# jkaardal/pyipm

Measured on AMD Instinct MI355X. Metric: newton_steps_per_sec, higher is better.
Workload: dtype f64

## Files before the change

### pyipm_amd/csrc/ctx.hpp

```cpp
#pragma once
#include <hip/hip_runtime.h>
#include <stdint.h>
#include <stdio.h>
#include <stdlib.h>
#include <string.h>
#include <string>
#include <new>
#include <stdexcept>
#include <map>
#include <memory>
#include <vector>
#include "../../include/pyipm_newton.h"
#include "owned.hpp"
#include "step_plan.hpp"

namespace pyipm {

constexpr int TB = PYIPM_TILE;
static_assert(TB == PLAN_TB, "step_plan.hpp states the tile on its own");
constexpr int PADG = PYIPM_PAD;
constexpr int BM = 128;
constexpr int BKU = 16;
constexpr int ROWCHUNK = 2048;

// ... 198 lines not shown
    struct TileList { unsigned* dev = nullptr; unsigned count = 0;
                      Event ready; hipStream_t on = nullptr; bool seen_done = false; };
    struct TlArena { DevBuf<unsigned> dev; PinnedBuf<unsigned> host{hipHostMallocDefault}; size_t used = 0; };
    std::vector<TlArena> tl_arenas;
    std::map<std::vector<int64_t>, TileList> tile_lists;
    int skip_zeros = 1;
    int group = 1;
    bool tail_group_user = false;
    int tail_group = 4;
    GroupSched sched;
    double* Wnext = nullptr;
    int group_chain = 1;
    Stream rest;
    std::vector<Event> ev_band;
    Event ev_join, ev_main, ev_split, ev_sfast;
    int keep_zeros = 1;
    int tile_step = 1;
    int sweep_max_blocks = 0;
    int occ_fwd_sweep = 0, occ_bwd_sweep = 0, occ_fwd_prefix = 0, occ_fwd_range = 0;
    int sweep_persist = 1;
    int bwd_slack = 1;
    DevBuf<double> sweep_buf;
    DevBuf<double> ms_buf;
    DevBuf<double> km_buf;
    int ms_matvec_many = 0;
    PollWords sweep_words{3 * 4096,
                          "backward sweep (k_bwd_sweep): a poll timed out in an earlier solve; its result was NaN"};
    int dist_slices = 2;
    double dist_timeout_s = 300.0;
    int dist_comm2 = 0;
// ... 157 lines not shown
```

### pyipm_amd/csrc/pyipm_newton.hip

```cpp
#include "driver.hpp"
#include "sub_walk.hpp"
#include "kernels_assemble.hpp"
#include "kernels_factor.hpp"
#include "kernels_panel.hpp"
#include "kernels_chain.hpp"
#include "kernels_solve.hpp"
#include "kernels_msolve.hpp"
#include "kernels_kmany.hpp"
#include "kernels_batched.hpp"
#include "kernels_merit.hpp"

using namespace pyipm;
using namespace pyipm::drv;

namespace pyipm { namespace drv {


size_t carve_workspace(Ctx* c, const Geo& g, char* base, bool provider_only = false) {
    Carve cv;
    const size_t D = sizeof(double);
    const size_t oA = cv.take(provider_only ? 256 : (size_t)g.Npad * (size_t)(g.ncols_local > 0 ? g.ncols_local : 1) * D);
    const size_t oW = cv.take(provider_only ? 256 : 3 * (size_t)default_group(g.world, g.nb) * (size_t)g.Npad * g.nb * D);
    const size_t oL = cv.take(g.world > 1 ? (size_t)g.Npad * g.nb * D : 256);
    const size_t oD = cv.take(provider_only ? 256 : (size_t)(g.Npad / TB) * TB * TB * D);
// ... 493 lines not shown
            hipLaunchKernelGGL(k_tile_step8, dim3(nblk), dim3(512), 0, chain, ctx->A, g.Npad, gc0, glc0, j, nT, ny, upb,
                               Wg, g.Npad, Dv, Ts, ctx->Tflag + gc0 / TB, ctx->refine_cond, ctx->block_refine, ctx->dstats, g.N,
                               ctx->pivtol_rel, ctx->anorm, g.n + g.mi, ctx->dbg_buf, ctx->tile_blocked);
            PYIPM_KCHECK();
            continue;
        }
        hipLaunchKernelGGL(k_tile_step, dim3((unsigned)(nT - j), (unsigned)ny), dim3(256), 0, chain, ctx->A, g.Npad, gc0, glc0, j,
                           Wg, g.Npad, Dv, Ts, ctx->Tflag + gc0 / TB, ctx->refine_cond, ctx->block_refine, ctx->dstats, g.N,
                           ctx->pivtol_rel, ctx->anorm, g.n + g.mi, ctx->dbg_buf, ctx->tile_blocked);
        PYIPM_KCHECK();
    }
    return 0;
}

struct SubPanel { int64_t c0, lc0; int nt; double* W; int64_t id; };
struct BlockDesc {
    std::vector<SubPanel> sp;
    bool wide = false;
    int64_t lp = 0;
    int64_t hole0 = 0, hole1 = 0;
};
int factor_block(Ctx* ctx, const BlockDesc& bd, hipStream_t chain, const std::function<int(int64_t, hipStream_t)>& on_done) {
    const Geo& g = ctx->g;
    const int64_t n0 = (int64_t)bd.sp.size();
    std::vector<int> toff((size_t)n0 + 1, 0);
    for (int64_t k = 0; k < n0; ++k) toff[(size_t)k + 1] = toff[(size_t)k] + bd.sp[(size_t)k].nt;
    const int nT = toff[(size_t)n0];
    const int64_t gc0 = bd.sp[0].c0, glc0 = bd.sp[0].lc0, gend = gc0 + (int64_t)nT * TB;
    const int64_t TT = (int64_t)TB * TB;
    { int r0 = ensure_rest_stream(ctx); if (r0) return r0; }
    PYIPM_HIP(ctx->ev_join.ensure(hipEventDisableTiming));
    PYIPM_HIP(ensure_events(ctx->ev_band, (size_t)n0, hipEventDisableTiming));
    double* Wg = bd.sp[0].W;
    double* Dv = ctx->Dinv + (gc0 / TB) * TT;
    double* Ts = ctx->Tsv + (gc0 / TB) * TT;
    auto upd = [&](hipStream_t st, const double* Lop, const double* Wop, int K, int64_t row_begin, int64_t k1, int64_t cnt,
                   int64_t src_c0) -> int {
        if (!bd.wide)
            return launch_update128(ctx, st, Lop, g.Npad, Wop, K, row_begin, bd.sp[(size_t)k1].id, cnt, {.bulk = false, .src_c0 = src_c0});
        const int s0 = (int)((bd.sp[(size_t)k1].c0 - g.panel_c0(bd.lp * g.world + g.rank)) / 128);
        const int nc = (int)((int64_t)(toff[(size_t)(k1 + cnt)] - toff[(size_t)k1]) * TB / 128);
        return launch_update128(ctx, st, Lop, g.Npad, Wop, K, row_begin, bd.lp, 1,
                                {.bulk = false, .src_c0 = src_c0, .sub0 = s0, .nct_sub = nc});
    };
    const bool one_launch = ctx->chain_whole && chain_applies(ctx, gc0, nT);
    ChainGeo cgw; memset(&cgw, 0, sizeof(cgw));
    if (one_launch) {
        PYIPM_HIP(hipEventRecord(ctx->ev_band[0], chain));
        PYIPM_HIP(hipStreamWaitEvent(ctx->rest, ctx->ev_band[0], 0));
        int r0 = launch_tile_steps(ctx, chain, gc0, glc0, nT, 0, nT, Wg, Dv, Ts); if (r0) return r0;
        cgw = ctx->chain_last;
    }
    for (int kp = 1, ta = 0; kp <= n0 && !one_launch; ++kp) {
        const int tb = kp < n0 ? toff[(size_t)kp] + 1 : nT;
        int r0 = launch_tile_steps(ctx, chain, gc0, glc0, nT, ta, tb, Wg, Dv, Ts); if (r0) return r0;
        if (kp < n0) PYIPM_HIP(hipEventRecord(ctx->ev_band[(size_t)(kp - 1)], chain));
        ta = tb;
    }
    for (int64_t k = 0; k < n0; ++k) {
        const SubPanel& q = bd.sp[(size_t)k];
        const int64_t c0 = q.c0, lc0 = q.lc0;
        const int nt = q.nt;
        hipStream_t rs = ctx->rest;
        if (k + 1 == n0) {
            PYIPM_HIP(hipEventRecord(ctx->ev_join, ctx->rest));
            PYIPM_HIP(hipStreamWaitEvent(chain, ctx->ev_join, 0));
            rs = chain;
        } else if (one_launch) {
            hipLaunchKernelGGL(k_chain_wait, dim3(1), dim3(64), 0, ctx->rest, cgw, toff[(size_t)k + 1], toff[(size_t)k + 1], toff[(size_t)k + 1]);
            PYIPM_KCHECK();
        } else {
            PYIPM_HIP(hipStreamWaitEvent(ctx->rest, ctx->ev_band[(size_t)k], 0));
        }
        const bool left = g.Npad - gend > PENDING_LEFT_ROWS;
        if (g.Npad > gend && left && k > 0) {
            const int K = toff[(size_t)k] * TB;
            int rc = upd(rs, ctx->A + glc0 * g.Npad, Wg, K, gend, k, 1, gc0);
            if (rc) return rc;
        }
        if (g.Npad > gend) {
            hipLaunchKernelGGL(k_panel_rest, dim3((unsigned)((g.Npad - gend) / TB)), dim3(256), 0, rs, ctx->A, g.Npad, c0, lc0, nt,
                               gend, q.W, g.Npad, ctx->Dinv + (c0 / TB) * TT, ctx->Tsv + (c0 / TB) * TT, ctx->Tflag + c0 / TB,
                               ctx->block_refine, bd.hole0, bd.hole1, &ctx->dstats->growth_bits);
            PYIPM_KCHECK();
            if (k + 1 < n0 && !left) {
                const int K = nt * TB;
                const SubPanel& nx = bd.sp[(size_t)k + 1];
                const int64_t tc0 = nx.c0, ncols = (int64_t)(nT - toff[(size_t)k + 1]) * TB;
                if (g.Npad - tc0 <= PENDING32_ROWS) {
                    int64_t pa0, pa1, pb0, pb1;
                    active_ranges(ctx, c0, c0 + K, &pa0, &pa1, &pb0, &pb1);
                    hipLaunchKernelGGL(k_inpanel_update, dim3((unsigned)((g.Npad - gend) / 32), (unsigned)(ncols / TB)), dim3(256), 0,
                                       rs, ctx->A, g.Npad, nx.lc0, ctx->A + lc0 * g.Npad, g.Npad, q.W, g.Npad,
                                       tc0, K, gend, g.Npad, pa0, pa1, pb0, pb1, SIDE_PRIO);
                    PYIPM_KCHECK();
                } else {
                    int rc = upd(rs, ctx->A + lc0 * g.Npad, q.W, K, gend, k + 1, n0 - 1 - k, c0);
                    if (rc) return rc;
                }
            }
        }
        if (one_launch && k + 1 < n0) {
            const int tq = toff[(size_t)k + 1] + 1;
            hipLaunchKernelGGL(k_chain_wait, dim3(1), dim3(64), 0, ctx->rest, cgw, tq, tq, tq);
            PYIPM_KCHECK();
        }
        int rc = on_done(q.id, rs); if (rc) return rc;
    }
    return 0;
}

int factor_group(Ctx* ctx, int64_t p0, int64_t n0, hipStream_t chain, const std::function<int(int64_t, hipStream_t)>& on_done) {
    const Geo& g = ctx->g;
    BlockDesc bd;
    for (int64_t k = 0; k < n0; ++k) {
        const int64_t q = p0 + k;
        bd.sp.push_back(SubPanel{g.panel_c0(q), g.local_c0(q), (int)(g.panel_w(q) / TB), wbuf(ctx, q), q});
    }
    if (ctx->skip_zeros && g.mi > 0 && ctx->sched.in_x_panel(p0)) slack_hole(g, &bd.hole0, &bd.hole1);
    return factor_block(ctx, bd, chain, on_done);
}

int factor_wide_panel(Ctx* ctx, int64_t p, hipStream_t stream) {
    const Geo& g = ctx->g;
    const int64_t c0 = g.panel_c0(p), lc0 = g.local_c0(p);
    const int nt = (int)(g.panel_w(p) / TB), snt = ctx->wide_sub / TB;
    BlockDesc bd;
    bd.wide = true; bd.lp = p / g.world;
    double* W = wbuf(ctx, p);
// ... 8 lines not shown
bool panel_is_wide(const Ctx* ctx, int64_t p) {
    return ctx->wide_sub >= 128 && ctx->wide_sub % 128 == 0 && ctx->g.panel_w(p) > ctx->wide_sub;
}
bool panel_piecewise_ok(const Ctx* ctx, int64_t p) {
    if (!ctx->tile_step || panel_in_s(ctx, p)) return false;
    const int nt = (int)ctx->g.panel_w(p) / TB;
    return panel_is_wide(ctx, p) ? (nt <= 32) : (nt <= 16);
}
int panel_chain(Ctx* ctx, int64_t p, hipStream_t stream, int64_t xrows, const unsigned* xword, unsigned xwant) {
    const Geo& g = ctx->g;
    const int64_t c0 = g.panel_c0(p), lc0 = g.local_c0(p);
    const int nt = (int)(g.panel_w(p) / TB);
    return launch_tile_steps(ctx, stream, c0, lc0, nt, 0, nt, wbuf(ctx, p), ctx->Dinv + (c0 / TB) * (int64_t)(TB * TB),
                             ctx->Tsv + (c0 / TB) * (int64_t)(TB * TB), (int)(xrows / TB), xword, xwant);
}
bool chain_extra_ok(const Ctx* ctx, int64_t p, int64_t xrows) {
    const Geo& g = ctx->g;
    const int64_t c0 = g.panel_c0(p);
    const int nbw = (int)g.panel_w(p), nt = nbw / TB;
    if (xrows <= 0 || xrows % TB != 0 || xrows / TB > 16 || c0 + nbw + xrows > g.Npad) return false;
    if (!(nt >= 2 && chain_applies(ctx, c0, nt))) return false;
    if (1 + 4 * (nt + (int)(xrows / TB)) > Ctx::CHAIN_WORDS) return false;
    int64_t h0 = 0, h1 = 0;
    panel_hole(ctx, p, &h0, &h1);
    const int64_t r0 = c0 + nbw, r1 = r0 + xrows;
    return !(h1 > h0 && r1 > h0 && r0 < h1);
}
int panel_rows(Ctx* ctx, int64_t p, int64_t r0, int64_t r1, hipStream_t stream) {
    const Geo& g = ctx->g;
    if (r1 > g.Npad) r1 = g.Npad;
    if (r1 <= r0) return 0;
    const int64_t c0 = g.panel_c0(p), lc0 = g.local_c0(p), TT = (int64_t)TB * TB;
    const int nbw = (int)g.panel_w(p), nt = nbw / TB;
    double* W = wbuf(ctx, p);
    int64_t hole0 = 0, hole1 = 0;
    panel_hole(ctx, p, &hole0, &hole1);
    if (!panel_is_wide(ctx, p)) {
        hipLaunchKernelGGL(k_panel_rest, dim3((unsigned)((r1 - r0) / TB)), dim3(256), 0, stream, ctx->A, g.Npad, c0, lc0, nt, r0,
                           W, g.Npad, ctx->Dinv + (c0 / TB) * TT, ctx->Tsv + (c0 / TB) * TT, ctx->Tflag + c0 / TB,
                           ctx->block_refine, hole0, hole1, &ctx->dstats->growth_bits);
        PYIPM_KCHECK();
// ... 885 lines not shown

static int panel_done(Ctx* ctx, const FactorRun& run, int64_t grp, int64_t q, hipStream_t used) {
    if (run.plan.fuse_forward && run.plan.fwd_owner(q, run.fr_blocks != 0) == FwdOwner::PanelDone) {
        const bool early = run.done_early(ctx, q);
        if (!early) PYIPM_HIP(hipEventRecord(ctx->ev_done[q], used));
        PYIPM_HIP(hipStreamWaitEvent(ctx->fwd, early && ctx->slack_one ? ctx->ev_sfast : ctx->ev_done[q], 0));
        const int r2 = fwd_panels(ctx, q, q + 1); if (r2) return r2;
    }
    if (!(run.plan.early0 && grp == 0)) return 0;
    const int64_t p1 = ctx->sched.first(1);
    PYIPM_HIP(hipEventRecord(ctx->ev_early, used));
    PYIPM_HIP(hipStreamWaitEvent(ctx->side, ctx->ev_early, 0));
    return timed_update(ctx, q, 1, p1, ctx->g.npanels - p1, {.stream = ctx->side, .as_bulk = true});
}

static int run_group(Ctx* ctx, const FactorRun& run, int64_t grp, hipStream_t S) {
    const int64_t pA = ctx->sched.first(grp), nA = ctx->sched.size(grp);
    auto done = [&](int64_t q, hipStream_t used) { return panel_done(ctx, run, grp, q, used); };
    if (chain_group(ctx, grp)) return factor_group(ctx, pA, nA, S, done);
    for (int64_t q = pA; q < pA + nA; ++q) {
        if (!run.done_early(ctx, q)) { int r2 = factor_panel(ctx, q, S, true); if (r2) return r2; }
        int r2 = done(q, S); if (r2) return r2;
    }
    return 0;
}

static int enqueue_slack_first(Ctx* ctx, const FactorRun& run, hipStream_t after) {
    { int r0 = ensure_rest_stream(ctx); if (r0) return r0; }
    PYIPM_HIP(hipEventRecord(ctx->ev_sfast, after));
    PYIPM_HIP(hipStreamWaitEvent(ctx->rest, ctx->ev_sfast, 0));
    const Geo& g = ctx->g;
    for (int64_t q = 0; q < g.npanels; ++q) {
        if (!ctx->sched.fast_panel(q)) continue;
        if (!ctx->slack_one) {
// ... 31 lines not shown
    }
    const int64_t rows = split ? cols : g.Npad - tc0;
    hipLaunchKernelGGL(k_inpanel_update, dim3((unsigned)(rows / 32), (unsigned)(cols / TB)), dim3(256), 0,
                       hs, ctx->A, g.Npad, g.local_c0(tp), ctx->A + g.local_c0(q0) * g.Npad, g.Npad,
                       wbuf(ctx, q0), g.Npad, tc0, K, tc0, g.Npad, pa0, pa1, pb0, pb1, SIDE_PRIO);
    PYIPM_KCHECK();
    if (below && g.Npad - tend <= HEAD32_ROWS) {
        hipLaunchKernelGGL(k_inpanel_update, dim3((unsigned)((g.Npad - tend) / 32), (unsigned)(cols / TB)), dim3(256), 0,
                           ctx->rest, ctx->A, g.Npad, g.local_c0(tp), ctx->A + g.local_c0(q0) * g.Npad, g.Npad,
                           wbuf(ctx, q0), g.Npad, tc0, K, tend, g.Npad, pa0, pa1, pb0, pb1, SIDE_PRIO);
        PYIPM_KCHECK();
    } else if (below) {
        return launch_update128(ctx, ctx->rest, ctx->A + g.local_c0(q0) * g.Npad, g.Npad, wbuf(ctx, q0), K, tend, tp, tn,
                                {.src_c0 = g.panel_c0(q0), .waves = HEAD_WAVES});
    }
    return 0;
}

struct GroupStep {
    bool fast_src, nxt_fast;
    bool across; int64_t pT, nT;
    bool pieces, head, split;
    hipStream_t cs, hs;
};
static GroupStep plan_step(const Ctx* ctx, const FactorRun& run, int64_t grp) {
    const GroupSched& sc = ctx->sched;
    GroupStep st; st.fast_src = sc.fast(grp); st.nxt_fast = sc.fast(grp + 1);
    st.cs = st.nxt_fast ? ctx->stream : ctx->side;
    st.across = run.plan.slack_first && st.nxt_fast && !st.fast_src && grp > 0 && grp + 2 < sc.ngroups() &&
                !sc.fast(grp + 2) && chain_group(ctx, grp + 2);
    st.pT = sc.first(grp + (st.across ? 2 : 1)); st.nT = sc.size(grp + (st.across ? 2 : 1));
    st.hs = (grp > 0 && (st.cs == ctx->side || st.across)) ? ctx->side : ctx->stream;
    st.pieces = run.plan.early0 && grp == 0;
    st.head = !st.pieces && (st.across || !st.nxt_fast);
    st.split = st.across || (chain_group(ctx, grp + 1) && st.cs != ctx->stream);
    return st;
}

static int enqueue_begin(Ctx* ctx, FactorRun& run) {
    const StepPlan& plan = run.plan;
    if (!ctx->side) {
        for (Event* e : {&ctx->ev_main, &ctx->ev_early, &ctx->ev_split, &ctx->ev_sfast})
            PYIPM_HIP(e->ensure(hipEventDisableTiming));
        PYIPM_HIP(ctx->side.ensure_highest(hipStreamNonBlocking));
    }
    PYIPM_HIP(hipEventRecord(ctx->ev[0], ctx->stream));
    ctx->held.factor_begun();
    if (plan.fuse_forward) {
        PYIPM_HIP(ctx->fwd.ensure(hipStreamNonBlocking));
        PYIPM_HIP(ensure_events(ctx->ev_done, (size_t)ctx->g.npanels, hipEventDisableTiming));
        PYIPM_HIP(hipEventRecord(ctx->ev_head, ctx->stream));
        PYIPM_HIP(hipStreamWaitEvent(ctx->fwd, ctx->ev_head, 0));
    }
    if (plan.kind != PX_REUSE) return factor_begin(ctx);
    const SnapHeaders hdr = snap_headers(ctx);
    PYIPM_HIP(hipMemcpyAsync(ctx->dstats, hdr.at_boundary, sizeof(DevStats), hipMemcpyDeviceToDevice, ctx->stream));
    if (plan.e.ok) { hipLaunchKernelGGL(k_merge_stats, dim3(1), dim3(64), 0, ctx->stream, ctx->dstats, (const DevStats*)hdr.of_lam_e); PYIPM_KCHECK(); }
// ... 60 lines not shown
        PYIPM_HIP(hipMemcpyAsync(hdr.of_lam_e, ctx->dstats, sizeof(DevStats), hipMemcpyDeviceToDevice, ctx->stream));
        hipLaunchKernelGGL(k_merge_stats, dim3(1), dim3(64), 0, ctx->stream, ctx->dstats, (const DevStats*)hdr.before_lam_e); PYIPM_KCHECK();
        rc = copy_square(ctx, lam_e_square(ctx, le), le.cE, true); if (rc) return rc;
    } else {
        rc = prefix_copy(ctx, plan, true); if (rc) return rc;
    }
    run.tr.mark(which == 2 ? "second snapshot end" : "snapshot end", grp, ctx->stream);
    rc = run_group(ctx, run, grp + 1, ctx->stream); if (rc) return rc;
    PYIPM_HIP(hipEventRecord(ctx->ev_main, ctx->stream));
    run.across_prev = false; return 0;
}
static int enqueue_groups(Ctx* ctx, FactorRun& run) {
    const StepPlan& plan = run.plan; const GroupSched& sc = ctx->sched; GroupTrace& tr = run.tr;
    const int64_t np = ctx->g.npanels, ngroups = sc.ngroups(), g0 = plan.g0; const bool reuse = plan.kind == PX_REUSE;
    if (reuse && plan.slack_first && sc.fast(g0)) PYIPM_HIP(hipStreamWaitEvent(ctx->stream, ctx->ev_sfast, 0));
    tr.mark("chain+rows begin", g0, ctx->stream);
    int rc = run_group(ctx, run, g0, ctx->stream); if (rc) return rc;
    tr.mark("chain+rows end", g0, ctx->stream);
    if (reuse) PYIPM_HIP(hipEventRecord(ctx->ev_main, ctx->stream));
    if (tr.on()) fprintf(stderr, "[pyipm group trace] %lld groups\n", (long long)ngroups);
    for (int64_t grp = g0; grp + 1 < ngroups; ++grp) {
        const int64_t p0 = sc.first(grp), n0 = sc.size(grp);
        const int snapshot = plan.snapshot_behind(grp);
        rc = record_behind(ctx, run, grp, snapshot); if (rc) return rc;
        if (snapshot) continue;
        if (!ctx->lookahead) {
            rc = timed_update(ctx, p0, n0, p0 + n0, np - (p0 + n0)); if (rc) return rc;
            rc = run_group(ctx, run, grp + 1, ctx->stream); if (rc) return rc;
            continue;
        }
        const GroupStep st = plan_step(ctx, run, grp);
        if (st.hs == ctx->side) {
            if (!run.across_prev) PYIPM_HIP(hipStreamWaitEvent(ctx->side, ctx->ev_main, 0));
            if (plan.slack_first && st.fast_src) PYIPM_HIP(hipStreamWaitEvent(ctx->side, ctx->ev_sfast, 0));
        }
        if (st.pieces) {
            PYIPM_HIP(hipEventRecord(ctx->ev_early, ctx->side));
            PYIPM_HIP(hipStreamWaitEvent(ctx->stream, ctx->ev_early, 0));
            if (ctx->rest) PYIPM_HIP(hipStreamWaitEvent(ctx->rest, ctx->ev_early, 0));
        } else {
            tr.mark("head begin", grp, st.hs);
            if (st.head) { rc = head_from(ctx, st.fast_src, p0, n0, st.pT, st.nT, st.hs, st.split); if (rc) return rc; }
            tr.mark("head end (its first launch's stream)", grp, st.hs);
        }
        if (st.hs == ctx->stream && st.cs == ctx->side) {
            PYIPM_HIP(hipEventRecord(ctx->ev_head, ctx->stream));
            PYIPM_HIP(hipStreamWaitEvent(ctx->side, ctx->ev_head, 0));
        }
        tr.mark("chain+rows begin", grp + 1, st.cs);
        if (plan.slack_first && st.nxt_fast)
            PYIPM_HIP(hipStreamWaitEvent(st.cs, ctx->ev_sfast, 0));
        if (plan.kind == PX_RECORD && plan.e.ok && grp + 1 == plan.e.gS) {
            PYIPM_HIP(hipMemcpyAsync(snap_headers(ctx).before_lam_e, ctx->dstats, sizeof(DevStats), hipMemcpyDeviceToDevice, st.cs));
            hipLaunchKernelGGL(k_init_stats, dim3(1), dim3(64), 0, st.cs, ctx->dstats); PYIPM_KCHECK();
        }
        rc = run_group(ctx, run, grp + 1, st.cs); if (rc) return rc;
        tr.mark("chain+rows end", grp + 1, st.cs);
        PYIPM_HIP(hipEventRecord(ctx->ev_panel, st.cs));
        tr.mark("bulk begin", grp, ctx->stream);
        if (!st.pieces) { rc = timed_update(ctx, p0, n0, st.pT + st.nT, np - (st.pT + st.nT)); if (rc) return rc; }
        tr.mark("bulk end", grp, ctx->stream);
        PYIPM_HIP(hipEventRecord(ctx->ev_main, ctx->stream));
        PYIPM_HIP(hipStreamWaitEvent(ctx->stream, ctx->ev_panel, 0));
        run.across_prev = st.across;
    }
    return 0;
}
static int enqueue_end(Ctx* ctx, FactorRun& run, pyipm_factor_stats* stats, std::chrono::steady_clock::time_point t_host0) {
    if (run.plan.fuse_forward) {
        run.tr.mark("fwd stream end (before group)", ctx->sched.ngroups(), ctx->fwd);
        PYIPM_HIP(hipEventRecord(ctx->ev_fwd, ctx->fwd));
        PYIPM_HIP(hipStreamWaitEvent(ctx->stream, ctx->ev_fwd, 0));
        ctx->held.forward_fused_under_factor();
    }
    PYIPM_HIP(hipEventRecord(ctx->ev[1], ctx->stream));
    ctx->held.factor_enqueued();
    if (getenv("PYIPM_SETUP_TRACE")) {
// ... 4 lines not shown
    const int rc = factor_end(ctx, stats);
    float ms = 0.f;
    PYIPM_HIP(hipEventElapsedTime(&ms, ctx->ev[0], ctx->ev[1]));
    run.tr.report(ctx->ev[0], ctx->ev[1], ms);
    ctx->t_factor = ms;
    ctx->t_panel = ctx->profile ? (ms - ctx->t_trailing_union) : 0.0;
    return rc;
}

int factor_all(Ctx* ctx, pyipm_factor_stats* stats, bool fuse_forward = false, int px = PX_FULL) {
    const Geo& g = ctx->g;
    if (g.world != 1) { ctx->err = "factor(): single-rank entry point; use the per-panel phases when world > 1"; return PYIPM_E_BADARG; }
    if (!ctx->held.assembled) { ctx->err = "factor: assemble first"; return PYIPM_E_BADARG; }
    const auto t_host0 = std::chrono::steady_clock::now();
    const SchedOpts o = sched_opts(ctx); ctx->sched = plan_groups(g, o);
    FactorRun run{make_step_plan(g, ctx->sched, o, px, px && ctx->held.plan.e.ok, fuse_forward, fwd_prefix_applies(ctx))};
    const StepPlan& plan = run.plan;
    if (px && plan.kind == PX_FULL) { ctx->err = "factor: no reusable prefix in this schedule"; return PYIPM_E_BADARG; }
    if (px && !(plan == ctx->held.plan && (!plan.e.ok || ctx->snap_e))) {
        const char* const what = plan.e.ok || ctx->held.plan.e.ok ? "lambda_e groups" : "x prefix";
        ctx->err = "factor: the schedule changed behind the assembly of a step that keeps the " + std::string(what); return PYIPM_E_BADARG;
    }
    if (plan.frB > plan.frA) run.fr_blocks = fwd_range_grid(ctx, plan.frA, plan.frB);
    if (run.tr.on()) {
        const bool rec = plan.kind == PX_RECORD, reuse = plan.kind == PX_REUSE;
        fprintf(stderr, "[pyipm group trace] %s step%s\n", rec ? "recording" : reuse ? "reusing" : "full",
                reuse ? ": the x-block prefix is kept" : "");
        if (px) fprintf(stderr, "[pyipm group trace] %s %lld groups: x prefix [0, %lld), lambda_e [%lld, %lld)\n", rec ? "records" : "keeps",
                        (long long)(plan.gB + (plan.e.ok ? plan.e.gE - plan.e.gS : 0)), (long long)plan.gB, (long long)plan.e.gS, (long long)plan.e.gE);
    }
    int rc = enqueue_begin(ctx, run); if (rc) return rc;
// ... 129 lines not shown
    ctx->device = device;
    ctx->stream = (hipStream_t)stream;
    if (hipSetDevice(device) != hipSuccess) return PYIPM_E_NODEVICE;
    set(ctx.get());
    const size_t need = carve(nullptr, nullptr);
    if (workspace) {
        if (workspace_bytes < need) return PYIPM_E_NOMEM;
        ctx->ws.adopt((char*)workspace, need);
    } else {
        if (ctx->ws.reserve(need) != hipSuccess) return PYIPM_E_NOMEM;
        if (getenv("PYIPM_POISON_WORKSPACE")) hipMemset(ctx->ws, 0xFF, need);
    }
    carve(ctx.get(), ctx->ws.get());
    if (hipMemset(ctx->anorm, 0, anorm_words * sizeof(unsigned long long)) != hipSuccess) return PYIPM_E_HIP;
    for (Event& e : ctx->ev) if (e.ensure(hipEventDefault) != hipSuccess) return PYIPM_E_HIP;
    if (schedule_events) {
        for (Event& e : ctx->ev_prov) if (e.ensure(hipEventDefault) != hipSuccess) return PYIPM_E_HIP;
        for (Event* e : {&ctx->ev_fwd, &ctx->ev_head, &ctx->ev_panel}) if (e->ensure(hipEventDisableTiming) != hipSuccess) return PYIPM_E_HIP;
    }
    *out = reinterpret_cast<pyipm_newton_ctx*>(ctx.release());
    return PYIPM_OK;
}

static int create_impl(pyipm_newton_ctx** out, int64_t n, int64_t me, int64_t mi, int nb, int device,
                       int world, int rank, void* workspace, size_t workspace_bytes, void* stream, bool provider_only) {
    if (nb == 0) nb = 256;
    const bool args_ok = n > 0 && me >= 0 && mi >= 0 && world >= 1 && rank >= 0 && rank < world && nb % 128 == 0 && nb <= 1024;
    const Geo g = args_ok ? make_geo(n, me, mi, nb, world, rank) : Geo{};
    return create_handle(out, args_ok, device, workspace, workspace_bytes, stream,
        [&](Ctx* ctx) {
            ctx->g = g;
            ctx->gc = make_geo(n, me, 0, nb, 1, 0);
            ctx->group = default_group(world, nb);
            { int ncu = 0; if (hipDeviceGetAttribute(&ncu, hipDeviceAttributeMultiprocessorCount, device) == hipSuccess && ncu > 0) ctx->num_cus = ncu; }
            ctx->provider_only = provider_only;
            { const char* e = getenv("PYIPM_REUSE_X"); if (e && e[0] == '0') ctx->reuse_x = 0; }
            { const char* e = getenv("PYIPM_REUSE_LAM_E"); if (e && e[0] == '0') ctx->reuse_lam_e = 0; }
            { const char* e = getenv("PYIPM_FWD_PREFIX"); if (e) { const int w = atoi(e); if (w <= 0) ctx->fwd_prefix = 0; else if (w >= 2) ctx->fwd_prefix_wgs = w; } }
            { const char* e = getenv("PYIPM_FWD_RANGE"); if (e) { const int w = atoi(e); if (w <= 0) ctx->fwd_range = 0; else if (w >= 2) ctx->fwd_range_wgs = w; } }
            { const char* e = getenv("PYIPM_SLACK_ONE"); if (e && atoi(e) <= 0) ctx->slack_one = 0; }
            { const char* e = getenv("PYIPM_BWD_SLACK"); if (e && e[0] == '0') ctx->bwd_slack = 0; }
            { const char* e = getenv("PYIPM_MS_MATVEC_MANY"); if (e && atoi(e) > 0) ctx->ms_matvec_many = 1; }
        },
        [&](Ctx* ctx, char* base) { return carve_workspace(ctx, g, base, provider_only); },
        2 , true);
}

int pyipm_newton_create(pyipm_newton_ctx** out, int64_t n, int64_t me, int64_t mi, int nb, int device,
                        int world, int rank, void* workspace, size_t workspace_bytes, void* stream) try {
    return create_impl(out, n, me, mi, nb, device, world, rank, workspace, workspace_bytes, stream, false);
} PYIPM_CATCH_NOH

size_t pyipm_newton_workspace_bytes_provider(int64_t n, int64_t me, int64_t mi) try {
    if (n <= 0 || me < 0 || mi < 0) return 0;
    Geo g = make_geo(n, me, mi, 256, 1, 0);
    return carve_workspace(nullptr, g, nullptr, true);
// ... 1217 lines not shown
```

### pyipm_amd/csrc/step_plan.hpp

```cpp
#pragma once
#include <cstddef>
#include <cstdint>
#include <vector>
namespace pyipm {
constexpr int PLAN_TB = 64;
constexpr int64_t TAIL_COLS = 24576;
constexpr int PX_HDR = 32;
constexpr int PX_HDR_SECOND = 16;

struct PlanGeo {
    int64_t n, me, mi, Npad; int nb; int64_t npanels;
    int64_t panel_c0(int64_t p) const { return p * (int64_t)nb; }
    int64_t panel_w(int64_t p) const { const int64_t w = Npad - p * (int64_t)nb; return w < nb ? w : nb; }
};
struct SchedOpts { int group, tail_group; bool tail_group_user, skip_zeros; int lookahead; bool group_chain; };

struct GroupSched {
    std::vector<int> of_, off_;
    std::vector<int64_t> first_;
    std::vector<char> fast_;
    std::vector<char> in_x_;
    bool active() const { return !of_.empty(); }
    void clear() { of_.clear(); off_.clear(); first_.clear(); fast_.clear(); in_x_.clear(); }
    bool has(int64_t p) const { return (size_t)p < of_.size(); }
// ... 62 lines not shown
    e.ok = true; e.gS = gS; e.gE = gE; e.cS = c0(gS); e.cE = c0(gE);
    return e;
}
inline size_t lam_e_doubles(const PlanGeo& g, const LamE& e) { const size_t rows = (size_t)(g.Npad - e.cE); return PX_HDR + rows * (size_t)(e.cE - e.cS) + rows * rows; }

enum class FwdOwner { Prefix, Range, Kept, PanelDone };
struct StepPlan {
    int kind = PX_FULL;
    int64_t gB = 0, cB = 0; LamE e;
    int64_t g0 = 0;
    bool early0 = false;
    bool slack_first = false;
    PxRange ranges[2] = {}; int nranges = 0; size_t snap_doubles = 0, snap_e_doubles = 0;
    bool fuse_forward = false, fwd_prefix_launch = false, fr_slack = false;
    int64_t pB = 0, pS = 0, pE = 0, frA = 0, frB = 0;
    bool operator==(const StepPlan& o) const {
        return kind == o.kind && gB == o.gB && cB == o.cB && e == o.e && g0 == o.g0 && early0 == o.early0 && slack_first == o.slack_first && snap_doubles == o.snap_doubles && snap_e_doubles == o.snap_e_doubles; }
    int snapshot_behind(int64_t grp) const { return kind != PX_RECORD ? 0 : (e.ok && grp + 1 == e.gE) ? 2 : grp + 1 == gB ? 1 : 0; }
    FwdOwner fwd_owner(int64_t q, bool range_used) const {
        return q < pB ? FwdOwner::Prefix : range_used && q >= frA && q < frB ? FwdOwner::Range : q >= pS && q < pE ? FwdOwner::Kept : FwdOwner::PanelDone;
    }
};
inline StepPlan make_step_plan(const PlanGeo& g, const GroupSched& sc, const SchedOpts& o, int kind, bool lam_e, bool fuse_forward, bool sweeps) {
    StepPlan p;
    const int64_t ng = sc.ngroups(), gB = prefix_groups(sc);
    if (kind != PX_FULL && gB > 0 && gB < ng && o.lookahead) {
        p.kind = kind; p.gB = gB; p.cB = g.panel_c0(sc.first(gB));
        if (lam_e) p.e = lam_e_groups(g, sc, gB);
        p.snap_doubles = prefix_ranges(g, p.cB, p.ranges, &p.nranges);
        if (p.e.ok) p.snap_e_doubles = lam_e_doubles(g, p.e);
// ... 1 lines not shown
    const bool reuse = p.kind == PX_REUSE;
    p.g0 = reuse ? (p.e.ok ? p.e.gE : gB) : 0;
    p.early0 = p.kind == PX_FULL && o.lookahead >= 2 && ng > 2 && chain_group(g, sc, o.group_chain, 0) && sc.fast(1);
    if (p.kind != PX_RECORD && o.lookahead && !sc.fast(0)) for (int64_t gi = 1; gi < ng; ++gi) p.slack_first = p.slack_first || sc.fast(gi);
    p.fuse_forward = fuse_forward;
    if (!reuse) return p;
    p.pB = p.pS = p.pE = sc.first(gB); if (p.e.ok) { p.pS = sc.first(p.e.gS); p.pE = sc.first(p.e.gE); }
    p.fwd_prefix_launch = fuse_forward && sweeps && p.pB >= 1 && p.pB * g.nb <= g.n;
    if (p.e.ok && p.fwd_prefix_launch) {
        p.fr_slack = p.slack_first;
        for (int64_t grp = gB; grp < p.e.gS; ++grp) p.fr_slack = p.fr_slack && sc.fast(grp);
        p.frA = p.fr_slack ? p.pB : p.pS; p.frB = p.pE;
    }
    return p;
}
}
```

Before: 176.1.

## Split tail groups so the chain factors the next group's diagonal rows early

Adds a tail-split schedule for the last chain groups in reuse mode. The head update is split into a diagonal part, an extra-rows part gated by a device flag word, and the remaining rows. The following group's chain launch also factors those extra rows, so the next diagonal block can start sooner. The bulk update is split so the next head's columns are released first. This aims to shorten the serial critical path near the end of factorization, at the cost of more events, flag polling, extra launches and complex cross-stream dependencies.

```diff
diff --git a/pyipm_amd/csrc/ctx.hpp b/pyipm_amd/csrc/ctx.hpp
--- a/pyipm_amd/csrc/ctx.hpp
+++ b/pyipm_amd/csrc/ctx.hpp
@@ -236,6 +236,10 @@
     Stream rest;
     std::vector<Event> ev_band;
     Event ev_join, ev_main, ev_split, ev_sfast;
+    int tail_split = 1;
+    Event ev_rows, ev_head2, ev_chain_end;
+    DevBuf<unsigned> tail_flag;
+    unsigned tail_token = 0;
     int keep_zeros = 1;
     int tile_step = 1;
     int sweep_max_blocks = 0;
diff --git a/pyipm_amd/csrc/pyipm_newton.hip b/pyipm_amd/csrc/pyipm_newton.hip
--- a/pyipm_amd/csrc/pyipm_newton.hip
+++ b/pyipm_amd/csrc/pyipm_newton.hip
@@ -531,11 +531,13 @@
 }
 
 struct SubPanel { int64_t c0, lc0; int nt; double* W; int64_t id; };
+struct TailHand { int64_t xrows = 0; const unsigned* xword = nullptr; unsigned xwant = 0; hipEvent_t rows_behind = nullptr; };
 struct BlockDesc {
     std::vector<SubPanel> sp;
     bool wide = false;
     int64_t lp = 0;
     int64_t hole0 = 0, hole1 = 0;
+    TailHand hand;
 };
 int factor_block(Ctx* ctx, const BlockDesc& bd, hipStream_t chain, const std::function<int(int64_t, hipStream_t)>& on_done) {
     const Geo& g = ctx->g;
@@ -561,12 +563,17 @@
                                 {.bulk = false, .src_c0 = src_c0, .sub0 = s0, .nct_sub = nc});
     };
     const bool one_launch = ctx->chain_whole && chain_applies(ctx, gc0, nT);
+    const bool hand = bd.hand.xrows > 0;
+    const int64_t rbeg = gend + bd.hand.xrows;
+    if (hand && !one_launch) { ctx->err = "factor_block: the tail split needs the one-launch chain (group_extra_ok)"; return PYIPM_E_BADARG; }
+    if (bd.hand.rows_behind) PYIPM_HIP(hipStreamWaitEvent(ctx->rest, bd.hand.rows_behind, 0));
     ChainGeo cgw; memset(&cgw, 0, sizeof(cgw));
     if (one_launch) {
         PYIPM_HIP(hipEventRecord(ctx->ev_band[0], chain));
         PYIPM_HIP(hipStreamWaitEvent(ctx->rest, ctx->ev_band[0], 0));
-        int r0 = launch_tile_steps(ctx, chain, gc0, glc0, nT, 0, nT, Wg, Dv, Ts); if (r0) return r0;
+        int r0 = launch_tile_steps(ctx, chain, gc0, glc0, nT, 0, nT, Wg, Dv, Ts, (int)(bd.hand.xrows / TB), bd.hand.xword, bd.hand.xwant); if (r0) return r0;
         cgw = ctx->chain_last;
+        if (hand) PYIPM_HIP(hipEventRecord(ctx->ev_chain_end, chain));
     }
     for (int kp = 1, ta = 0; kp <= n0 && !one_launch; ++kp) {
         const int tb = kp < n0 ? toff[(size_t)kp] + 1 : nT;
@@ -579,7 +586,7 @@
         const int64_t c0 = q.c0, lc0 = q.lc0;
         const int nt = q.nt;
         hipStream_t rs = ctx->rest;
-        if (k + 1 == n0) {
+        if (k + 1 == n0 && !hand) {
             PYIPM_HIP(hipEventRecord(ctx->ev_join, ctx->rest));
             PYIPM_HIP(hipStreamWaitEvent(chain, ctx->ev_join, 0));
             rs = chain;
@@ -590,14 +597,14 @@
             PYIPM_HIP(hipStreamWaitEvent(ctx->rest, ctx->ev_band[(size_t)k], 0));
         }
         const bool left = g.Npad - gend > PENDING_LEFT_ROWS;
-        if (g.Npad > gend && left && k > 0) {
+        if (g.Npad > rbeg && left && k > 0) {
             const int K = toff[(size_t)k] * TB;
-            int rc = upd(rs, ctx->A + glc0 * g.Npad, Wg, K, gend, k, 1, gc0);
+            int rc = upd(rs, ctx->A + glc0 * g.Npad, Wg, K, rbeg, k, 1, gc0);
             if (rc) return rc;
         }
-        if (g.Npad > gend) {
-            hipLaunchKernelGGL(k_panel_rest, dim3((unsigned)((g.Npad - gend) / TB)), dim3(256), 0, rs, ctx->A, g.Npad, c0, lc0, nt,
-                               gend, q.W, g.Npad, ctx->Dinv + (c0 / TB) * TT, ctx->Tsv + (c0 / TB) * TT, ctx->Tflag + c0 / TB,
+        if (g.Npad > rbeg) {
+            hipLaunchKernelGGL(k_panel_rest, dim3((unsigned)((g.Npad - rbeg) / TB)), dim3(256), 0, rs, ctx->A, g.Npad, c0, lc0, nt,
+                               rbeg, q.W, g.Npad, ctx->Dinv + (c0 / TB) * TT, ctx->Tsv + (c0 / TB) * TT, ctx->Tflag + c0 / TB,
                                ctx->block_refine, bd.hole0, bd.hole1, &ctx->dstats->growth_bits);
             PYIPM_KCHECK();
             if (k + 1 < n0 && !left) {
@@ -607,29 +614,35 @@
                 if (g.Npad - tc0 <= PENDING32_ROWS) {
                     int64_t pa0, pa1, pb0, pb1;
                     active_ranges(ctx, c0, c0 + K, &pa0, &pa1, &pb0, &pb1);
-                    hipLaunchKernelGGL(k_inpanel_update, dim3((unsigned)((g.Npad - gend) / 32), (unsigned)(ncols / TB)), dim3(256), 0,
+                    hipLaunchKernelGGL(k_inpanel_update, dim3((unsigned)((g.Npad - rbeg) / 32), (unsigned)(ncols / TB)), dim3(256), 0,
                                        rs, ctx->A, g.Npad, nx.lc0, ctx->A + lc0 * g.Npad, g.Npad, q.W, g.Npad,
-                                       tc0, K, gend, g.Npad, pa0, pa1, pb0, pb1, SIDE_PRIO);
+                                       tc0, K, rbeg, g.Npad, pa0, pa1, pb0, pb1, SIDE_PRIO);
                     PYIPM_KCHECK();
                 } else {
-                    int rc = upd(rs, ctx->A + lc0 * g.Npad, q.W, K, gend, k + 1, n0 - 1 - k, c0);
+                    int rc = upd(rs, ctx->A + lc0 * g.Npad, q.W, K, rbeg, k + 1, n0 - 1 - k, c0);
                     if (rc) return rc;
                 }
             }
         }
-        if (one_launch && k + 1 < n0) {
+        if (one_launch && k + 1 < n0 && !hand) {
             const int tq = toff[(size_t)k + 1] + 1;
             hipLaunchKernelGGL(k_chain_wait, dim3(1), dim3(64), 0, ctx->rest, cgw, tq, tq, tq);
             PYIPM_KCHECK();
         }
+        if (hand) continue;
         int rc = on_done(q.id, rs); if (rc) return rc;
     }
-    return 0;
-}
-
-int factor_group(Ctx* ctx, int64_t p0, int64_t n0, hipStream_t chain, const std::function<int(int64_t, hipStream_t)>& on_done) {
-    const Geo& g = ctx->g;
-    BlockDesc bd;
+    if (hand) {
+        PYIPM_HIP(hipStreamWaitEvent(ctx->rest, ctx->ev_chain_end, 0));
+        for (int64_t k = 0; k < n0; ++k) { int rc = on_done(bd.sp[(size_t)k].id, ctx->rest); if (rc) return rc; }
+        PYIPM_HIP(hipEventRecord(ctx->ev_rows, ctx->rest));
+    }
+    return 0;
+}
+
+int factor_group(Ctx* ctx, int64_t p0, int64_t n0, hipStream_t chain, const std::function<int(int64_t, hipStream_t)>& on_done, const TailHand& hand = {}) {
+    const Geo& g = ctx->g;
+    BlockDesc bd; bd.hand = hand;
     for (int64_t k = 0; k < n0; ++k) {
         const int64_t q = p0 + k;
         bd.sp.push_back(SubPanel{g.panel_c0(q), g.local_c0(q), (int)(g.panel_w(q) / TB), wbuf(ctx, q), q});
@@ -668,17 +681,27 @@
     return launch_tile_steps(ctx, stream, c0, lc0, nt, 0, nt, wbuf(ctx, p), ctx->Dinv + (c0 / TB) * (int64_t)(TB * TB),
                              ctx->Tsv + (c0 / TB) * (int64_t)(TB * TB), (int)(xrows / TB), xword, xwant);
 }
-bool chain_extra_ok(const Ctx* ctx, int64_t p, int64_t xrows) {
-    const Geo& g = ctx->g;
-    const int64_t c0 = g.panel_c0(p);
-    const int nbw = (int)g.panel_w(p), nt = nbw / TB;
+static bool block_extra_ok(const Ctx* ctx, int64_t c0, int nt, int64_t xrows, int64_t h0, int64_t h1) {
+    const Geo& g = ctx->g;
+    const int64_t nbw = (int64_t)nt * TB;
     if (xrows <= 0 || xrows % TB != 0 || xrows / TB > 16 || c0 + nbw + xrows > g.Npad) return false;
     if (!(nt >= 2 && chain_applies(ctx, c0, nt))) return false;
     if (1 + 4 * (nt + (int)(xrows / TB)) > Ctx::CHAIN_WORDS) return false;
+    const int64_t r0 = c0 + nbw, r1 = r0 + xrows;
+    return !(h1 > h0 && r1 > h0 && r0 < h1);
+}
+bool chain_extra_ok(const Ctx* ctx, int64_t p, int64_t xrows) {
     int64_t h0 = 0, h1 = 0;
     panel_hole(ctx, p, &h0, &h1);
-    const int64_t r0 = c0 + nbw, r1 = r0 + xrows;
-    return !(h1 > h0 && r1 > h0 && r0 < h1);
+    return block_extra_ok(ctx, ctx->g.panel_c0(p), (int)ctx->g.panel_w(p) / TB, xrows, h0, h1);
+}
+static bool group_extra_ok(const Ctx* ctx, int64_t grp, int64_t xrows) {
+    const Geo& g = ctx->g;
+    const int64_t p0 = ctx->sched.first(grp), p1 = ctx->sched.first(grp + 1);
+    int64_t cols = 0, h0 = 0, h1 = 0;
+    for (int64_t q = p0; q < p1; ++q) cols += g.panel_w(q);
+    if (ctx->skip_zeros && g.mi > 0 && ctx->sched.in_x_panel(p0)) slack_hole(g, &h0, &h1);
+    return ctx->chain_whole && cols / TB <= 32 && block_extra_ok(ctx, g.panel_c0(p0), (int)(cols / TB), xrows, h0, h1);
 }
 int panel_rows(Ctx* ctx, int64_t p, int64_t r0, int64_t r1, hipStream_t stream) {
     const Geo& g = ctx->g;
@@ -1594,10 +1617,10 @@
     return timed_update(ctx, q, 1, p1, ctx->g.npanels - p1, {.stream = ctx->side, .as_bulk = true});
 }
 
-static int run_group(Ctx* ctx, const FactorRun& run, int64_t grp, hipStream_t S) {
+static int run_group(Ctx* ctx, const FactorRun& run, int64_t grp, hipStream_t S, const TailHand& hand = {}) {
     const int64_t pA = ctx->sched.first(grp), nA = ctx->sched.size(grp);
     auto done = [&](int64_t q, hipStream_t used) { return panel_done(ctx, run, grp, q, used); };
-    if (chain_group(ctx, grp)) return factor_group(ctx, pA, nA, S, done);
+    if (chain_group(ctx, grp)) return factor_group(ctx, pA, nA, S, done, hand);
     for (int64_t q = pA; q < pA + nA; ++q) {
         if (!run.done_early(ctx, q)) { int r2 = factor_panel(ctx, q, S, true); if (r2) return r2; }
         int r2 = done(q, S); if (r2) return r2;
@@ -1659,6 +1682,26 @@
         return launch_update128(ctx, ctx->rest, ctx->A + g.local_c0(q0) * g.Npad, g.Npad, wbuf(ctx, q0), K, tend, tp, tn,
                                 {.src_c0 = g.panel_c0(q0), .waves = HEAD_WAVES});
     }
+    return 0;
+}
+
+__global__ __launch_bounds__(64) void k_tail_mark(unsigned* p, unsigned v) { if (threadIdx.x == 0) __hip_atomic_store(p, v, __ATOMIC_RELAXED, __HIP_MEMORY_SCOPE_AGENT); }
+static int head_split(Ctx* ctx, GroupTrace& tr, int64_t grp, int64_t q0, int64_t nq, int64_t tp, int64_t tn, hipStream_t ds, int64_t xnext) {
+    const Geo& g = ctx->g; const bool release = xnext > 0;
+    int K = 0; int64_t cols = 0;
+    for (int64_t q = q0; q < q0 + nq; ++q) K += (int)g.panel_w(q);
+    for (int64_t q = tp; q < tp + tn; ++q) cols += g.panel_w(q);
+    const int64_t tc0 = g.panel_c0(tp), tend = tc0 + cols, src = g.panel_c0(q0);
+    const double* Lop = ctx->A + g.local_c0(q0) * g.Npad;
+    int rc = launch_update128(ctx, ds, Lop, g.Npad, wbuf(ctx, q0), K, tc0, tp, tn, {.row_end = tend, .src_c0 = src, .prio = SIDE_PRIO}); if (rc) return rc;
+    tr.mark("diag head end", grp, ds);
+    PYIPM_HIP(hipStreamWaitEvent(ctx->stream, ctx->ev_rows, 0));
+    const int64_t xend = release ? tend + xnext : tend;
+    if (xend > tend) { rc = launch_update128(ctx, ctx->stream, Lop, g.Npad, wbuf(ctx, q0), K, tend, tp, tn, {.row_end = xend, .src_c0 = src}); if (rc) return rc; }
+    if (release) { hipLaunchKernelGGL(k_tail_mark, dim3(1), dim3(64), 0, ctx->stream, ctx->tail_flag.get(), ++ctx->tail_token); PYIPM_KCHECK(); }
+    if (xend < g.Npad) { rc = launch_update128(ctx, ctx->stream, Lop, g.Npad, wbuf(ctx, q0), K, xend, tp, tn, {.src_c0 = src}); if (rc) return rc; }
+    PYIPM_HIP(hipEventRecord(ctx->ev_head2, ctx->stream));
+    tr.mark("rest of head end", grp, ctx->stream);
     return 0;
 }
 
@@ -1685,7 +1728,7 @@
 static int enqueue_begin(Ctx* ctx, FactorRun& run) {
     const StepPlan& plan = run.plan;
     if (!ctx->side) {
-        for (Event* e : {&ctx->ev_main, &ctx->ev_early, &ctx->ev_split, &ctx->ev_sfast})
+        for (Event* e : {&ctx->ev_main, &ctx->ev_early, &ctx->ev_split, &ctx->ev_sfast, &ctx->ev_rows, &ctx->ev_head2, &ctx->ev_chain_end})
             PYIPM_HIP(e->ensure(hipEventDisableTiming));
         PYIPM_HIP(ctx->side.ensure_highest(hipStreamNonBlocking));
     }
@@ -1776,8 +1819,14 @@
     const StepPlan& plan = run.plan; const GroupSched& sc = ctx->sched; GroupTrace& tr = run.tr;
     const int64_t np = ctx->g.npanels, ngroups = sc.ngroups(), g0 = plan.g0; const bool reuse = plan.kind == PX_REUSE;
     if (reuse && plan.slack_first && sc.fast(g0)) PYIPM_HIP(hipStreamWaitEvent(ctx->stream, ctx->ev_sfast, 0));
+    auto hand_of = [&](int64_t h, bool gated) {
+        TailHand th;
+        if (plan.split(h)) { th.xrows = group_cols(ctx->g, sc, h + 1); if (gated) { th.xword = ctx->tail_flag.get(); th.xwant = ctx->tail_token; } }
+        if (gated) th.rows_behind = ctx->ev_head2;
+        return th;
+    };
     tr.mark("chain+rows begin", g0, ctx->stream);
-    int rc = run_group(ctx, run, g0, ctx->stream); if (rc) return rc;
+    int rc = run_group(ctx, run, g0, ctx->stream, hand_of(g0, false)); if (rc) return rc;
     tr.mark("chain+rows end", g0, ctx->stream);
     if (reuse) PYIPM_HIP(hipEventRecord(ctx->ev_main, ctx->stream));
     if (tr.on()) fprintf(stderr, "[pyipm group trace] %lld groups\n", (long long)ngroups);
@@ -1800,10 +1849,17 @@
             PYIPM_HIP(hipEventRecord(ctx->ev_early, ctx->side));
             PYIPM_HIP(hipStreamWaitEvent(ctx->stream, ctx->ev_early, 0));
             if (ctx->rest) PYIPM_HIP(hipStreamWaitEvent(ctx->rest, ctx->ev_early, 0));
+        } else if (plan.split(grp)) {
+            tr.mark("head begin", grp, st.cs);
+            rc = head_split(ctx, tr, grp, p0, n0, st.pT, st.nT, st.cs, plan.split(grp + 1) ? group_cols(ctx->g, sc, grp + 2) : 0); if (rc) return rc;
         } else {
             tr.mark("head begin", grp, st.hs);
             if (st.head) { rc = head_from(ctx, st.fast_src, p0, n0, st.pT, st.nT, st.hs, st.split); if (rc) return rc; }
             tr.mark("head end (its first launch's stream)", grp, st.hs);
+            if (plan.split(grp + 1)) {
+                PYIPM_HIP(hipEventRecord(ctx->ev_head2, ctx->rest));
+                PYIPM_HIP(hipStreamWaitEvent(st.cs, ctx->ev_head2, 0));
+            }
         }
         if (st.hs == ctx->stream && st.cs == ctx->side) {
             PYIPM_HIP(hipEventRecord(ctx->ev_head, ctx->stream));
@@ -1816,13 +1872,19 @@
             PYIPM_HIP(hipMemcpyAsync(snap_headers(ctx).before_lam_e, ctx->dstats, sizeof(DevStats), hipMemcpyDeviceToDevice, st.cs));
             hipLaunchKernelGGL(k_init_stats, dim3(1), dim3(64), 0, st.cs, ctx->dstats); PYIPM_KCHECK();
         }
-        rc = run_group(ctx, run, grp + 1, st.cs); if (rc) return rc;
+        rc = run_group(ctx, run, grp + 1, st.cs, hand_of(grp + 1, plan.split(grp))); if (rc) return rc;
         tr.mark("chain+rows end", grp + 1, st.cs);
         PYIPM_HIP(hipEventRecord(ctx->ev_panel, st.cs));
         tr.mark("bulk begin", grp, ctx->stream);
-        if (!st.pieces) { rc = timed_update(ctx, p0, n0, st.pT + st.nT, np - (st.pT + st.nT)); if (rc) return rc; }
+        const int64_t nA = plan.split(grp) && grp + 2 < ngroups ? sc.size(grp + 2) : 0;
+        if (nA > 0) {
+            rc = timed_update(ctx, p0, n0, st.pT + st.nT, nA); if (rc) return rc;
+            PYIPM_HIP(hipEventRecord(ctx->ev_main, ctx->stream));
+            tr.mark("bulk, next head's columns end", grp, ctx->stream);
+        }
+        if (!st.pieces) { rc = timed_update(ctx, p0, n0, st.pT + st.nT + nA, np - (st.pT + st.nT + nA)); if (rc) return rc; }
         tr.mark("bulk end", grp, ctx->stream);
-        PYIPM_HIP(hipEventRecord(ctx->ev_main, ctx->stream));
+        if (nA == 0) PYIPM_HIP(hipEventRecord(ctx->ev_main, ctx->stream));
         PYIPM_HIP(hipStreamWaitEvent(ctx->stream, ctx->ev_panel, 0));
         run.across_prev = st.across;
     }
@@ -1857,7 +1919,9 @@
     if (!ctx->held.assembled) { ctx->err = "factor: assemble first"; return PYIPM_E_BADARG; }
     const auto t_host0 = std::chrono::steady_clock::now();
     const SchedOpts o = sched_opts(ctx); ctx->sched = plan_groups(g, o);
-    FactorRun run{make_step_plan(g, ctx->sched, o, px, px && ctx->held.plan.e.ok, fuse_forward, fwd_prefix_applies(ctx))};
+    StepPlan decided = make_step_plan(g, ctx->sched, o, px, px && ctx->held.plan.e.ok, fuse_forward, fwd_prefix_applies(ctx));
+    plan_tail_split(decided, g, ctx->sched, o, ctx->tail_split != 0, HEAD32_ROWS, [&](int64_t grp, int64_t rows) { return group_extra_ok(ctx, grp, rows); });
+    FactorRun run{std::move(decided)};
     const StepPlan& plan = run.plan;
     if (px && plan.kind == PX_FULL) { ctx->err = "factor: no reusable prefix in this schedule"; return PYIPM_E_BADARG; }
     if (px && !(plan == ctx->held.plan && (!plan.e.ok || ctx->snap_e))) {
@@ -2017,6 +2081,10 @@
     carve(ctx.get(), ctx->ws.get());
     if (hipMemset(ctx->anorm, 0, anorm_words * sizeof(unsigned long long)) != hipSuccess) return PYIPM_E_HIP;
     for (Event& e : ctx->ev) if (e.ensure(hipEventDefault) != hipSuccess) return PYIPM_E_HIP;
+    if (ctx->tail_split) {
+        if (ctx->tail_flag.reserve(1) != hipSuccess) return PYIPM_E_NOMEM;
+        if (hipMemset(ctx->tail_flag.get(), 0, sizeof(unsigned)) != hipSuccess || hipDeviceSynchronize() != hipSuccess) return PYIPM_E_HIP;
+    }
     if (schedule_events) {
         for (Event& e : ctx->ev_prov) if (e.ensure(hipEventDefault) != hipSuccess) return PYIPM_E_HIP;
         for (Event* e : {&ctx->ev_fwd, &ctx->ev_head, &ctx->ev_panel}) if (e->ensure(hipEventDisableTiming) != hipSuccess) return PYIPM_E_HIP;
@@ -2043,6 +2111,7 @@
             { const char* e = getenv("PYIPM_FWD_RANGE"); if (e) { const int w = atoi(e); if (w <= 0) ctx->fwd_range = 0; else if (w >= 2) ctx->fwd_range_wgs = w; } }
             { const char* e = getenv("PYIPM_SLACK_ONE"); if (e && atoi(e) <= 0) ctx->slack_one = 0; }
             { const char* e = getenv("PYIPM_BWD_SLACK"); if (e && e[0] == '0') ctx->bwd_slack = 0; }
+            { const char* e = getenv("PYIPM_TAIL_SPLIT"); if (e && e[0] == '0') ctx->tail_split = 0; }
             { const char* e = getenv("PYIPM_MS_MATVEC_MANY"); if (e && atoi(e) > 0) ctx->ms_matvec_many = 1; }
         },
         [&](Ctx* ctx, char* base) { return carve_workspace(ctx, g, base, provider_only); },
diff --git a/pyipm_amd/csrc/step_plan.hpp b/pyipm_amd/csrc/step_plan.hpp
--- a/pyipm_amd/csrc/step_plan.hpp
+++ b/pyipm_amd/csrc/step_plan.hpp
@@ -100,6 +100,8 @@
     PxRange ranges[2] = {}; int nranges = 0; size_t snap_doubles = 0, snap_e_doubles = 0;
     bool fuse_forward = false, fwd_prefix_launch = false, fr_slack = false;
     int64_t pB = 0, pS = 0, pE = 0, frA = 0, frB = 0;
+    std::vector<char> tail_split;
+    bool split(int64_t grp) const { return grp >= 0 && (size_t)grp < tail_split.size() && tail_split[(size_t)grp] != 0; }
     bool operator==(const StepPlan& o) const {
         return kind == o.kind && gB == o.gB && cB == o.cB && e == o.e && g0 == o.g0 && early0 == o.early0 && slack_first == o.slack_first && snap_doubles == o.snap_doubles && snap_e_doubles == o.snap_e_doubles; }
     int snapshot_behind(int64_t grp) const { return kind != PX_RECORD ? 0 : (e.ok && grp + 1 == e.gE) ? 2 : grp + 1 == gB ? 1 : 0; }
@@ -131,4 +133,90 @@
     }
     return p;
 }
-}
+
+inline int64_t group_cols(const PlanGeo& g, const GroupSched& sc, int64_t grp) {
+    int64_t w = 0; for (int64_t q = sc.first(grp); q < sc.first(grp + 1); ++q) w += g.panel_w(q); return w;
+}
+template <class ExtraOk>
+inline void plan_tail_split(StepPlan& p, const PlanGeo& g, const GroupSched& sc, const SchedOpts& o, bool on, int64_t tail_rows, ExtraOk extra_ok) {
+    const int64_t ng = sc.ngroups();
+    p.tail_split.assign((size_t)ng, 0);
+    if (!on || p.kind != PX_REUSE || !o.lookahead || p.early0) return;
+    for (int64_t grp = p.g0; grp + 1 < ng; ++grp)
+        p.tail_split[(size_t)grp] = chain_group(g, sc, o.group_chain, grp) && chain_group(g, sc, o.group_chain, grp + 1) &&
+                                    g.Npad - g.panel_c0(sc.first(grp + 1)) <= tail_rows &&
+                                    extra_ok(grp, group_cols(g, sc, grp + 1));
+}
+enum TailItem {
+    TI_CHAIN,
+    TI_XROWS,
+    TI_ROWS,
+    TI_HEAD_DIAG,
+    TI_HEAD_XROWS,
+    TI_HEAD_REST,
+    TI_HEAD_OLD,
+    TI_BULK_NEXT,
+    TI_BULK_REST,
+    TI_COUNT
+};
+struct TailRegion { int item; int64_t src, dst, r0, r1; };
+struct TailDep { int reader, writer, rel; const char* by; };
+constexpr TailDep TAIL_DEPS[] = {
+    {TI_XROWS, TI_CHAIN, 0, "same launch: the chain's progress words"},
+    {TI_ROWS, TI_CHAIN, 0, "k_chain_wait on ctx->rest (pieces: ev_band); the last sub-panel where h is not split: ev_join"},
+    {TI_HEAD_DIAG, TI_XROWS, 0, "stream order behind the chain's launch; ev_main where the source ran on the main stream"},
+    {TI_HEAD_XROWS, TI_XROWS, 0, "ev_rows, recorded behind ev_chain_end"},
+    {TI_HEAD_XROWS, TI_ROWS, 0, "ev_rows"},
+    {TI_HEAD_REST, TI_XROWS, 0, "ev_rows, recorded behind ev_chain_end"},
+    {TI_HEAD_REST, TI_ROWS, 0, "ev_rows"},
+    {TI_HEAD_OLD, TI_ROWS, 0, "stream order: the last rows kernel runs on the chain's stream behind ev_join (ev_main behind group g0)"},
+    {TI_HEAD_OLD, TI_CHAIN, 0, "stream order (a source that is no chain group)"},
+    {TI_BULK_NEXT, TI_ROWS, 0, "ev_rows, then the main stream's order behind the head"},
+    {TI_BULK_REST, TI_ROWS, 0, "split: as TI_BULK_NEXT; else ev_panel of the iteration before (ev_main / stream order behind g0)"},
+    {TI_BULK_REST, TI_CHAIN, 0, "stream order / ev_panel (a source that is no chain group)"},
+    {TI_CHAIN, TI_HEAD_DIAG, 1, "stream order (the chain's stream)"},
+    {TI_CHAIN, TI_HEAD_OLD, 1, "stream order (the chain's stream; ev_head where the head ran on the main stream)"},
+    {TI_XROWS, TI_HEAD_XROWS, 1, "the flag word, set behind that launch and enqueued before the chain that polls it"},
+    {TI_XROWS, TI_HEAD_OLD, 1, "ev_head2 recorded on ctx->rest behind the old head, waited for by the chain's stream"},
+    {TI_ROWS, TI_HEAD_REST, 1, "ev_head2"},
+    {TI_ROWS, TI_HEAD_OLD, 1, "stream order on ctx->rest (ev_split), or the chain's stream"},
+    {TI_HEAD_DIAG, TI_BULK_NEXT, 1, "ev_main, recorded behind that launch"},
+    {TI_HEAD_DIAG, TI_BULK_REST, 1, "ev_main"},
+    {TI_HEAD_XROWS, TI_BULK_NEXT, 1, "the main stream's order"},
+    {TI_HEAD_XROWS, TI_BULK_REST, 1, "the main stream's order"},
+    {TI_HEAD_REST, TI_BULK_NEXT, 1, "the main stream's order"},
+    {TI_HEAD_REST, TI_BULK_REST, 1, "the main stream's order"},
+    {TI_HEAD_OLD, TI_BULK_NEXT, 1, "ev_main, recorded behind that launch"},
+    {TI_HEAD_OLD, TI_BULK_REST, 1, "ev_main"},
+    {TI_BULK_NEXT, TI_BULK_REST, 1, "the main stream's order"},
+    {TI_BULK_REST, TI_BULK_REST, 1, "the main stream's order"},
+};
+inline const TailDep* tail_dep(int reader, int writer, int rel) {
+    for (const TailDep& d : TAIL_DEPS) if (d.reader == reader && d.writer == writer && d.rel == rel) return &d;
+    return nullptr;
+}
+inline std::vector<TailRegion> tail_regions(const StepPlan& p, const PlanGeo& g, const GroupSched& sc, const SchedOpts& o, int64_t from) {
+    std::vector<TailRegion> v;
+    const int64_t ng = sc.ngroups();
+    auto c0 = [&](int64_t h) { return h >= ng ? g.Npad : g.panel_c0(sc.first(h)); };
+    for (int64_t h = from; h < ng; ++h) {
+        const int64_t a = c0(h), b = c0(h + 1), x = p.split(h) ? c0(h + 2) : b;
+        if (!chain_group(g, sc, o.group_chain, h)) { v.push_back({TI_CHAIN, h, h, a, g.Npad}); }
+        else {
+            v.push_back({TI_CHAIN, h, h, a, b});
+            if (x > b) v.push_back({TI_XROWS, h, h, b, x});
+            if (g.Npad > x) v.push_back({TI_ROWS, h, h, x, g.Npad});
+        }
+        if (h + 1 >= ng) continue;
+        if (p.split(h)) {
+            const int64_t t0 = b, t1 = c0(h + 2), xe = p.split(h + 1) ? c0(h + 3) : t1;
+            v.push_back({TI_HEAD_DIAG, h, h + 1, t0, t1});
+            if (xe > t1) v.push_back({TI_HEAD_XROWS, h, h + 1, t1, xe});
+            if (g.Npad > xe) v.push_back({TI_HEAD_REST, h, h + 1, xe, g.Npad});
+        } else v.push_back({TI_HEAD_OLD, h, h + 1, b, g.Npad});
+        for (int64_t c = h + 2; c < ng; ++c)
+            v.push_back({p.split(h) && c == h + 2 ? TI_BULK_NEXT : TI_BULK_REST, h, c, c0(c), g.Npad});
+    }
+    return v;
+}
+}
```

Result: faster. 185.3 (median of 6 runs) (+5.2%).
